# cvlab-stonybrook/s-volsdf

Measured on AMD Instinct MI355X. Metric: rendered rays/sec (1024-ray batch, 128 samples), higher is better.
Workload: dtype f32 (every product, forward and backward, as three fp16 MFMA products of two-piece fp16 operands with f32 accumulate; activation blocks hold both pieces: float32 accuracy class); 1 GPU; configs[1]: VolOpt.train_step (forward + MVS prior lookup + loss + backward + clip/guard/Adam), train mode, fast=1: 1024 rays/GPU x 128 coarse + 98 composited samples + 2048 eikonal points, 8x256 SDF MLP + 4x256 radiance MLP; mode=train, mlp_precision=fp16x2, launch=eager launches, rays_per_gpu=1024, rays_total=1024

## Files before the change

### s-volsdf_amd/csrc/svs_mlp_bwd_h2.hip

```cpp
#include "svs_mlp_h2_dev.h"
#include "svs_mlp_host.h"
#include "svs_mlp_bwd_args.h"
#include "svs_mlp_h2_trunk.h"
#include "svs_mlp_bwd_h2_dev.h"
#include "svs_ticket.h"
#include <cstdlib>

namespace svs {
namespace mlp {

template <bool GP>
struct RgbBwdEpi {
  f32x16 prev;
  TilePieces r;
  float v8[8];
  Pieces2* out;
  float* zblk;
  PointScale* ps;
  int lane;
  __device__ __forceinline__ void b(int tp, int rr) {
    float v = prev[rr] * ps->inv_in;
    v = hi_at(r, rr) > 0.0f ? v : 0.0f;
    pin(v);
    ps->track(v);
    v8[rr & 7] = v * ps->s_out;
    if ((rr & 7) == 7) {
      split8(v8, out->h[2 * tp + (rr >> 3)], out->m[2 * tp + (rr >> 3)]);
      pin(out->h[2 * tp + (rr >> 3)], out->m[2 * tp + (rr >> 3)]);
    }
    if (rr == 9) store_piece(zblk, 2 * tp, lane, out->h[2 * tp], 0);
    if (GP && rr == 11) store_piece(zblk, 2 * tp, lane, out->m[2 * tp], 1);
    if (rr == 15) store_grad<GP>(zblk, 2 * tp + 1, lane, out->h[2 * tp + 1], out->m[2 * tp + 1]);
  }
  __device__ __forceinline__ void all(int tp) {
#pragma unroll
    for (int rr = 0; rr < 16; ++rr) b(tp, rr);
  }
};

template <bool GP>
__device__ __forceinline__ void rgb_bwd_layer_h2(Stream& st, const Pieces2& in, Pieces2& out, const float* rblk, float* zblk,
                                                 float* zrec, PointScale& ps, int lane) {
  RgbBwdEpi<GP> ep;
  ep.out = &out; ep.zblk = zblk; ep.ps = &ps; ep.lane = lane;
  store_record(zrec, lane, ps.s_out, 0.0f);
  TilePieces rnext;
  load_tile_hi(rblk, 0, lane, rnext);
#pragma unroll
  for (int t = 0; t < 8; ++t) {
    const TilePieces rcur = rnext;
    auto rload = [&](int s) {
      if (t == 7) return;
      if (s == 10) rnext.h[0] = load_piece(rblk, 2 * (t + 1), lane);
      if (s == 12) rnext.h[1] = load_piece(rblk, 2 * (t + 1) + 1, lane);
    };
    f32x16 acc;
    if (t == 0) acc = tile_mma_h2_pf<16, kChunkF4>(st, in, lane, NoEpi(), NoEpi(), rload);
    else acc = tile_mma_h2_pf<16, kChunkF4>(st, in, lane, NoEpi(), [&](int s) { ep.b(t - 1, s); }, rload);
    ep.prev = acc; ep.r = rcur;
    constexpr int kSt = GP ? 4 : 2;
    if (t == 0) st.advance_keep<2>();
    else if (t < 7) st.advance_keep<2 + kSt>();
    else st.advance_keep<kSt>();
  }
  ep.all(7);
  ps.next();
}

template <bool GP>
__global__ __launch_bounds__(kThreads, 1) void rgb_bwd_h2_kernel(RgbBwdArgs a) {
  extern __shared__ __attribute__((aligned(16))) unsigned char smem[];
  Stream st;
  st.g = a.stream; st.buf = reinterpret_cast<f32x4*>(smem); st.cur = 1;
  const int lane = threadIdx.x & 63, half = lane >> 5, wave = threadIdx.x >> 6;
  const int wtile = blockIdx.x * kWaves + wave;
  const int p = wtile * kTilePts + (lane & 31);
  const bool livep = p < a.P;
  const int pc = livep ? p : a.P - 1;
  const size_t LS = block_stride();
  const float* rb = a.rbuf + (size_t)wtile * kBlockF;
  float* zb = a.zbuf + (size_t)wtile * kBlockF;
  const size_t T = (size_t)gridDim.x * kWaves;
  auto zrec = [&](int l) { return record_ptr(a.zbuf, 5, T, l, wtile); };

  st.prefetch<kW4TF4>();
  float dz[3];
  float m0 = 0.0f;
#pragma unroll
  for (int c = 0; c < 3; ++c) {
    const float o = a.rgb[3 * pc + c];
    dz[c] = (livep && half == 0) ? a.d_rgb[3 * pc + c] * o * (1.0f - o) : 0.0f;
    m0 = __builtin_fmaxf(m0, __builtin_fabsf(dz[c]));
  }
  m0 = __builtin_fmaxf(m0, __shfl_xor(m0, 32));
  PointScale ps;
  ps.start(m0, 0.0f);
  {
    float v8[8] = {dz[0] * ps.s_in, dz[1] * ps.s_in, dz[2] * ps.s_in, 0.0f, 0.0f, 0.0f, 0.0f, 0.0f};
    store_grad8<GP>(zb + 4 * LS, 0, lane, v8);
    store_record(zrec(4), lane, ps.s_in, m0);
  }
  st.advance();
  Pieces2 pa, pb;
  st.prefetch<kChunkF4>();
  {
    const f32x4* c = st.cur_buf();
    const float* r4 = rb + 3 * LS;
    float* z3 = zb + 3 * LS;
    store_record(zrec(3), lane, ps.s_out, 0.0f);
#pragma unroll
    for (int t = 0; t < 8; ++t) {
      TilePieces r;
      load_tile_hi(r4, t, lane, r);
      const f32x4 w = c[t * 64 + lane];
      f32x16 acc = (f32x16)(0.0f);
      acc = __builtin_amdgcn_mfma_f32_32x32x2f32(w[0], dz[0], acc, 0, 0, 0);
      acc = __builtin_amdgcn_mfma_f32_32x32x2f32(w[1], dz[1], acc, 0, 0, 0);
      acc = __builtin_amdgcn_mfma_f32_32x32x2f32(w[2], dz[2], acc, 0, 0, 0);
#pragma unroll
      for (int i = 0; i < 16; ++i) { acc[i] = hi_at(r, i) > 0.0f ? acc[i] : 0.0f; ps.track(acc[i]); }
      split_tile_scaled(acc, t, pa, ps.s_out);
      store_grad<GP>(z3, 2 * t, lane, pa.h[2 * t], pa.m[2 * t]);
      store_grad<GP>(z3, 2 * t + 1, lane, pa.h[2 * t + 1], pa.m[2 * t + 1]);
    }
  }
  ps.next();
  st.advance();
  rgb_bwd_layer_h2<GP>(st, pa, pb, rb + 2 * LS, zb + 2 * LS, zrec(2), ps, lane);
  rgb_bwd_layer_h2<GP>(st, pb, pa, rb + 1 * LS, zb + 1 * LS, zrec(1), ps, lane);
  rgb_bwd_layer_h2<GP>(st, pa, pb, rb, zb, zrec(0), ps, lane);
  float* fb = a.feat_bar + (size_t)wtile * kBlockF;
  float fmax = 0.0f;
  const float s_f = ps.s_out;
  {
    f32x16 prev;
    float v8[8];
    auto slice = [&](int tp, int r) {
      const float v = prev[r] * ps.inv_in;
      fmax = __builtin_fmaxf(fmax, __builtin_fabsf(v));
      v8[r & 7] = v * s_f;
      if ((r & 7) == 7) store_grad8<GP>(fb, 2 * tp + (r >> 3), lane, v8);
    };
#pragma unroll
    for (int t = 0; t < 9; ++t) {
      if (t < 8) st.prefetch<kChunkF4>();
      f32x16 acc;
      if (t == 0) acc = tile_mma_h2<16>(st.cur_buf(), pb, lane);
      else acc = tile_mma_h2<16>(st.cur_buf(), pb, lane, NoEpi(), [&](int s) { slice(t - 1, s); });
      if (t < 8) { prev = acc; st.advance(); }
      else if (half == 1 && livep) {
        a.d_normals[3 * p] = acc[4] * ps.inv_in; a.d_normals[3 * p + 1] = acc[5] * ps.inv_in;
        a.d_normals[3 * p + 2] = acc[6] * ps.inv_in;
      }
    }
  }
  fmax = __builtin_fmaxf(fmax, __shfl_xor(fmax, 32));
  store_record(record_ptr(a.feat_bar, 1, T, 0, wtile), lane, s_f, fmax);
  publish_max(a.absmax + 1, ps.gmax);
  publish_max(a.absmax + 2, fmax);
}

constexpr int kSpliceF = 20;

template <bool SPLIT, bool GP>
struct PassAEpi {
  f32x16 prev;
  TilePieces h;
  float v, s1;
  float v8[8];
  f16x8 up[2], uq[2];
  Pieces2* out;
  float* ublk;
  float* urec;
  PointScale* ps;
  const float* splice;
  float vm;
  int lane, half;
  bool l3;

  __device__ __forceinline__ void begin() {
    if (lane < 32) urec[lane] = ps->s_out;
    vm = 0.0f;
  }
  __device__ __forceinline__ void end() {
    vm = __builtin_fmaxf(vm, __shfl_xor(vm, 32));
    if (lane >= 32) urec[lane] = vm;
  }
  __device__ __forceinline__ void a(int r) {
    v = prev[r] * ps->inv_in;
    s1 = 1.0f - __builtin_amdgcn_exp2f(grad_times<GP>(h, r, -100.0f * 1.44269504088896341f));
    pin(v); pin(s1);
  }
  template <bool LATE = false>
  __device__ __forceinline__ void b(int tp, int r) {
    float u = v * s1;
    float w = __builtin_fabsf(v) * (100.0f - 100.0f * s1);
    if (tp == 6 && r >= 12 && l3) {
      const bool sp = half == 1 || r >= 13;
      const float us = splice[(16 + (r - 12)) * kThreads];
      u = sp ? us : u;
      w = sp ? 0.0f : w;
    }
    pin(u); pin(w);
    emit<LATE>(tp, r, u, w);
  }
  template <bool LATE = false>
  __device__ __forceinline__ void emit(int tp, int r, float u, float w) {
    vm = __builtin_fmaxf(vm, w);
    ps->track(u);
    v8[r & 7] = u * ps->s_out;
    if ((r & 7) == 7) {
      const int k = 2 * tp + (r >> 3), q = r >> 3;
      if (SPLIT) {
        split8(v8, out->h[k], out->m[k]);
        pin(out->h[k], out->m[k]);
        up[q] = out->h[k];
        if (GP) uq[q] = out->m[k];
      } else if (GP) {
        split8(v8, up[q], uq[q]);
      } else {
        up[q] = hi8(v8, 1.0f);
      }
      if (!LATE) store_grad<GP>(ublk, k, lane, up[q], uq[q]);
    }
  }
  __device__ __forceinline__ void store_slot(int tp, int s) {
    if (s == 9) store_piece(ublk, 2 * tp, lane, up[0], 0);
    if (GP && s == 11) store_piece(ublk, 2 * tp, lane, uq[0], 1);
    if (s == 15) store_grad<GP>(ublk, 2 * tp + 1, lane, up[1], uq[1]);
  }
  __device__ __forceinline__ void all(int tp) {
#pragma unroll
    for (int r = 0; r < 16; ++r) { a(r); b(tp, r); }
  }
  __device__ __forceinline__ void splice_tile7() {
#pragma unroll
    for (int r = 0; r < 16; ++r) emit(7, r, splice[r * kThreads], 0.0f);
  }
};

template <bool SPLIT, bool LAST, bool GP>
__device__ __forceinline__ void pass_a_layer_h2(Stream& st, const Pieces2& in, PassAEpi<SPLIT, GP>& ep, const float* hblk, int lane) {
  ep.begin();
#pragma unroll
  for (int t = 0; t < 8; ++t) {
    if (t == 7 && ep.l3) break;
    TilePieces hload;
    load_tile_grad<GP>(hblk, t, lane, hload);
    const bool fetch = !(LAST && t == 7);
    f32x16 acc;
    if (!fetch) acc = tile_mma_h2<16>(st.cur_buf(), in, lane, [&](int s) { ep.a(s); }, [&](int s) { ep.b(t - 1, s); });
    else if (t == 0) acc = tile_mma_h2_pf<16, kChunkF4>(st, in, lane, NoEpi(), NoEpi());
    else acc = tile_mma_h2_pf<16, kChunkF4>(st, in, lane, [&](int s) { ep.a(s); },
                                            [&](int s) { ep.template b<true>(t - 1, s); ep.store_slot(t - 1, s); });
    ep.prev = acc; ep.h = hload;
    if (fetch) {
      if (t == 0) st.advance();
      else st.advance_keep<GP ? 4 : 2>();
    }
  }
  if (ep.l3) { ep.all(6); ep.splice_tile7(); }
  else ep.all(7);
  ep.end();
  ep.ps->next();
}

template <bool GP>
__global__ __launch_bounds__(kThreads, 1) void sdf_bwd_a_h2_kernel(SdfBwdAArgs a) {
  extern __shared__ __attribute__((aligned(16))) unsigned char smem[];
  Stream st;
  st.g = a.stream; st.buf = reinterpret_cast<f32x4*>(smem); st.cur = 1;
  float* splice = reinterpret_cast<float*>(smem + kLdsBytes) + threadIdx.x;
  const int lane = threadIdx.x & 63, half = lane >> 5, wave = threadIdx.x >> 6;
  const int wtile = blockIdx.x * kWaves + wave;
  const int p = wtile * kTilePts + (lane & 31);
  const int pc = p < a.src.P ? p : a.src.P - 1;

  st.prefetch<kChunk0F4>();
  PointScale ps;
  Pieces2 pa, pb;
  const size_t LS = block_stride();
  const float* hb = a.hbuf + (size_t)wtile * kBlockF;
  float* ub = a.ubuf + (size_t)wtile * kBlockF;
  const size_t T = (size_t)gridDim.x * kWaves;
  auto urec = [&](int l) { return record_ptr(a.ubuf, 9, T, l, wtile); };
  {
    float x0, x1, x2;
    load_point(a.src, p, x0, x1, x2);
    PosEnc pe;
    pe.compute(x0, x1, x2);
    float nb[3] = {a.d_grad[3 * pc], a.d_grad[3 * pc + 1], a.d_grad[3 * pc + 2]};
    if (p >= a.src.P || (a.clamp_mask && a.clamp_mask[pc])) { nb[0] = nb[1] = nb[2] = 0.0f; }
    PosEnc u0;
    float m0 = 0.0f;
#pragma unroll
    for (int q = 0; q < 40; ++q) {
      float coef = 1.0f; int c = q;
      if (q >= 3 && q < kPeDim) {
        const int f = (q - 3) / 6, w = (q - 3) % 6;
        const float sc = (float)(1 << f);
        c = w < 3 ? w : w - 3;
        coef = w < 3 ? sc * pe.v[q + 3] : -sc * pe.v[q - 3];
      }
      u0.v[q] = q < kPeDim ? coef * nb[c < 3 ? c : 0] : 0.0f;
      m0 = __builtin_fmaxf(m0, __builtin_fabsf(u0.v[q]));
    }
    ps.start(m0, 0.0f);
#pragma unroll
    for (int r = 0; r < 16; ++r) splice[r * kThreads] = half ? u0.v[rho(r) + 4] : u0.v[rho(r)];
#pragma unroll
    for (int r = 12; r < 16; ++r) {
      const int k0 = rho(r) - 25, k1 = rho(r) + 4 - 25;
      const float s0 = k0 >= 0 ? u0.v[32 + (k0 >= 0 ? k0 : 0)] : 0.0f;
      splice[(16 + r - 12) * kThreads] = half ? u0.v[32 + k1] : s0;
    }
    PosEnc us;
#pragma unroll
    for (int q = 0; q < 40; ++q) us.v[q] = u0.v[q] * ps.s_in;
    split_pe(us, half, pa);
    float* pbk = a.pebuf + (size_t)wtile * kBlockF;
#pragma unroll
    for (int k = 0; k < 3; ++k) {
      f16x8 fh, fm;
      block_fragment<kPeDim>(u0.v, k, half, ps.s_in, fh, fm);
      store_grad<GP>(ub, k, lane, fh, fm);
      block_fragment<kPeDim>(pe.v, k, half, 1.0f, fh, fm);
      store_grad<GP>(pbk, k, lane, fh, fm);
    }
    store_record(urec(0), lane, ps.s_in, m0);
  }
  st.advance();

  {
    PassAEpi<true, GP> ep;
    ep.out = &pb; ep.ublk = ub + LS; ep.urec = urec(1); ep.ps = &ps; ep.splice = splice;
    ep.lane = lane; ep.half = half; ep.l3 = false;
    ep.begin();
#pragma unroll
    for (int t = 0; t < 8; ++t) {
      TilePieces hload;
      load_tile_grad<GP>(hb, t, lane, hload);
      if (t < 7) st.prefetch<kChunk0F4>(); else st.prefetch<kChunkF4>();
      const f32x16 acc = tile_mma_h2<3>(st.cur_buf(), pa, lane);
      if (t > 0) ep.all(t - 1);
      ep.prev = acc; ep.h = hload;
      st.advance();
    }
    ep.all(7);
    ep.end();
    ps.next();
  }
  for (int l = 1; l < 7; ++l) {
    PassAEpi<true, GP> ep;
    ep.out = &pa; ep.ublk = ub + (size_t)(l + 1) * LS; ep.urec = urec(l + 1);
    ep.ps = &ps; ep.splice = splice; ep.lane = lane; ep.half = half; ep.l3 = l == 3;
    pass_a_layer_h2<true, false, GP>(st, pb, ep, hb + (size_t)l * LS, lane);
#pragma unroll
    for (int s = 0; s < 16; ++s) { pb.h[s] = pa.h[s]; pb.m[s] = pa.m[s]; }
  }
  {
    PassAEpi<false, GP> ep;
    ep.out = nullptr; ep.ublk = ub + (size_t)8 * LS; ep.urec = urec(8);
    ep.ps = &ps; ep.splice = splice; ep.lane = lane; ep.half = half; ep.l3 = false;
    pass_a_layer_h2<false, true, GP>(st, pb, ep, hb + (size_t)7 * LS, lane);
  }
  publish_max(a.absmax, ps.gmax);
}

template <bool FIRST, bool SPLIT, typename Net, bool A2, bool GP>
struct PassBEpi {
  static constexpr bool kG = A2 || FIRST;
  f32x16 prev;
  TilePieces h, u, g;
  float v, s1, q;
  float v8[8];
  f16x8 ap[2], aq[2];
  Pieces2* out;
  float* ablk;
  float* arec;
  PointScale* ps;
  float sbar, u_inv100;
  int lane, half;
  bool l4;
  __device__ __forceinline__ void a(int r) {
    v = prev[r] * ps->inv_in;
    float e = __builtin_amdgcn_exp2f(grad_times<GP>(h, r, -100.0f * 1.44269504088896341f));
    if (A2) e = __builtin_fminf(e, 0.99999994f);
    s1 = 1.0f - e;
    if (A2) q = e * u_inv100;
    pin(v); pin(s1);
    if (A2) pin(q);
  }
  template <bool LATE = false>
  __device__ __forceinline__ void b(int tp, int r) {
    float o = v * s1;
    if (A2) {
      const float gg = grad_mix<GP>(g, r);
      const float t = grad_times<GP>(u, r, gg);
      o = __builtin_fmaf(t, q * __builtin_amdgcn_rcpf(s1), o);
      if (FIRST) o = __builtin_fmaf(sbar, gg, o);
    } else if (FIRST) {
      o = __builtin_fmaf(sbar, grad_mix<GP>(g, r), o);
    }
    if (l4 && tp > Net::kSpliceTile) o = 0.0f;
    if (l4 && tp == Net::kSpliceTile) {
      const bool z0 = rho(r) >= Net::kSpliceLocal, z1 = rho(r) + 4 >= Net::kSpliceLocal;
      if (z0 || z1) { if (half ? z1 : z0) o = 0.0f; }
    }
    pin(o);
    ps->track(o);
    v8[r & 7] = o * ps->s_out;
    if ((r & 7) == 7) {
      const int k = 2 * tp + (r >> 3), q2 = r >> 3;
      if (SPLIT) {
        split8(v8, out->h[k], out->m[k]);
        pin(out->h[k], out->m[k]);
        ap[q2] = out->h[k];
        if (GP) aq[q2] = out->m[k];
      } else if (GP) {
        split8(v8, ap[q2], aq[q2]);
      } else {
        ap[q2] = hi8(v8, 1.0f);
      }
      if (!LATE) store_grad<GP>(ablk, k, lane, ap[q2], aq[q2]);
    }
  }
  __device__ __forceinline__ void store_slot(int tp, int s) {
    if (s == 9) store_grad<GP>(ablk, 2 * tp, lane, ap[0], aq[0]);
    if (s == 15) store_grad<GP>(ablk, 2 * tp + 1, lane, ap[1], aq[1]);
  }
  __device__ __forceinline__ void all(int tp) {
#pragma unroll
    for (int r = 0; r < 16; ++r) { a(r); b(tp, r); }
  }
};

template <bool FIRST, bool SPLIT, bool LAST_STAGE, typename Net, bool A2, bool GP>
__device__ __forceinline__ void pass_b_stage_h2(Stream& st, const Pieces2& in, PassBEpi<FIRST, SPLIT, Net, A2, GP>& ep, const float* hblk,
                                                const float* ublk, const float* urec, const float* gblk, float next_floor, int lane) {
  constexpr bool kG = A2 || FIRST;
  store_record(ep.arec, lane, ep.ps->s_out, 0.0f);
  ep.u_inv100 = A2 ? 100.0f * PointScale::inv_pow2(load_scale(urec, lane)) : 0.0f;
  TilePieces hnext, unext, gnext;
  load_tile_grad<GP>(hblk, 0, lane, hnext);
  if (A2) load_tile_grad<GP>(ublk, 0, lane, unext);
  if (kG) load_tile_grad<GP>(gblk, 0, lane, gnext);
  constexpr int kPer = GP ? 4 : 2;
  constexpr int kLoads = kPer * (1 + (A2 ? 1 : 0) + (kG ? 1 : 0));
  constexpr int kStores = GP ? 4 : 2;
#pragma unroll
  for (int t = 0; t < 8; ++t) {
    const TilePieces hcur = hnext, ucur = unext, gcur = gnext;
    auto side = [&](int s) {
      if (t == 7) return;
      if (s == 10) hnext.h[0] = load_piece(hblk, 2 * (t + 1), lane);
      if (s == 11) hnext.h[1] = load_piece(hblk, 2 * (t + 1) + 1, lane);
      if (A2 && s == 12) unext.h[0] = load_piece(ublk, 2 * (t + 1), lane);
      if (A2 && s == 13) unext.h[1] = load_piece(ublk, 2 * (t + 1) + 1, lane);
      if (kG && s == 14) gnext.h[0] = load_piece(gblk, 2 * (t + 1), lane);
      if (kG && s == 15) gnext.h[1] = load_piece(gblk, 2 * (t + 1) + 1, lane);
      if (GP) {
        if (s == 10) hnext.m[0] = load_piece(hblk, 2 * (t + 1), lane, 1);
        if (s == 11) hnext.m[1] = load_piece(hblk, 2 * (t + 1) + 1, lane, 1);
        if (A2 && s == 12) unext.m[0] = load_piece(ublk, 2 * (t + 1), lane, 1);
        if (A2 && s == 13) unext.m[1] = load_piece(ublk, 2 * (t + 1) + 1, lane, 1);
        if (kG && s == 14) gnext.m[0] = load_piece(gblk, 2 * (t + 1), lane, 1);
        if (kG && s == 15) gnext.m[1] = load_piece(gblk, 2 * (t + 1) + 1, lane, 1);
      }
    };
    const bool fetch = !(LAST_STAGE && t == 7);
    f32x16 acc;
    if (!fetch) acc = tile_mma_h2<16>(st.cur_buf(), in, lane, [&](int s) { ep.a(s); }, [&](int s) { ep.b(t - 1, s); });
    else if (t == 0) acc = tile_mma_h2_pf<16, kChunkF4>(st, in, lane, NoEpi(), NoEpi(), side);
    else acc = tile_mma_h2_pf<16, kChunkF4>(st, in, lane, [&](int s) { ep.a(s); },
                                            [&](int s) { ep.template b<true>(t - 1, s); ep.store_slot(t - 1, s); }, side);
    ep.prev = acc; ep.h = hcur;
    if (A2) ep.u = ucur;
    if (kG) ep.g = gcur;
    if (fetch) {
      if (t == 0) st.advance_keep<kLoads>();
      else if (t < 7) st.advance_keep<kLoads + kStores>();
      else st.advance_keep<kStores>();
    }
  }
  ep.all(7);
  ep.ps->floor_m = next_floor;
  ep.ps->next();
}

template <typename Net, bool A2, bool GP>
__global__ __launch_bounds__(kThreads, 1) void sdf_bwd_b_h2_kernel(SdfBwdBArgs a) {
  extern __shared__ __attribute__((aligned(16))) unsigned char smem[];
  Stream st;
  st.g = a.stream; st.buf = reinterpret_cast<f32x4*>(smem); st.cur = 1;
  const int lane = threadIdx.x & 63, half = lane >> 5, wave = threadIdx.x >> 6;
  const int bx = a.reverse ? (int)(gridDim.x - 1 - blockIdx.x) : (int)blockIdx.x;
  const int wtile = bx * kWaves + wave;
  const int p = wtile * kTilePts + (lane & 31);
  const int pc = p < a.P ? p : a.P - 1;
  st.prefetch<kChunkF4>();
  float sbar = (a.d_sdf && p < a.P) ? a.d_sdf[pc] : 0.0f;
  if (a.clamp_mask && a.clamp_mask[pc]) sbar = 0.0f;
  if (half == 0 && a.sbar_out) a.sbar_out[p] = sbar;
  const size_t LS = block_stride();
  const float* hb = a.hbuf + (size_t)wtile * kBlockF;
  const float* gb = A2 ? a.gbuf + (size_t)wtile * kBlockF : a.w0 + (size_t)wtile * a.w0_stride - 7 * LS;
  const float* ub = A2 ? a.ubuf + (size_t)wtile * kBlockF : nullptr;
  float* ab = a.abuf + (size_t)wtile * kBlockF;
  const size_t T = (size_t)gridDim.x * kWaves;
  auto arec = [&](int l) { return record_ptr(a.abuf, 8, T, l, wtile); };
  auto urec = [&](int l) { return A2 ? record_ptr(a.ubuf, 9, T, l, wtile) : nullptr; };
  const float asb = __builtin_fabsf(sbar);
  auto floor_of = [&](int l) {
    return A2 ? __builtin_fmaxf(asb, load_max(urec(l + 1), lane) * load_max(record_ptr(a.gbuf, 8, T, l, wtile), lane)) : asb;
  };
  const bool has_f = a.feat_bar && wtile < a.n_feat_tiles;
  PointScale ps;
  Pieces2 pa, pb;
  {
    const float fl = floor_of(7);
    if (has_f) {
      const float* fb = a.feat_bar + (size_t)wtile * kBlockF;
      const float* frec = record_ptr(a.feat_bar, 1, (size_t)((a.n_feat_tiles + kWaves - 1) / kWaves * kWaves), 0, wtile);
#pragma unroll
      for (int k = 0; k < 16; ++k) {
        pa.h[k] = load_piece(fb, k, lane);
        pa.m[k] = GP ? load_piece(fb, k, lane, 1) : (f16x8)(_Float16)0.0f;
      }
      ps.start_stored(load_scale(frec, lane), load_max(frec, lane), fl);
    } else {
#pragma unroll
      for (int k = 0; k < 16; ++k) { pa.h[k] = (f16x8)(_Float16)0.0f; pa.m[k] = (f16x8)(_Float16)0.0f; }
      ps.start(0.0f, fl);
    }
    ps.gmax = 0.0f;
  }
  st.advance();
  {
    PassBEpi<true, true, Net, A2, GP> ep;
    ep.out = &pb; ep.ablk = ab + 7 * LS; ep.arec = arec(7); ep.ps = &ps; ep.sbar = sbar; ep.lane = lane; ep.half = half; ep.l4 = false;
    pass_b_stage_h2<true, true, false, Net, A2, GP>(st, pa, ep, hb + 7 * LS, A2 ? ub + 8 * LS : nullptr, urec(8), gb + 7 * LS,
                                                    floor_of(6), lane);
  }
  for (int l = 7; l >= 2; --l) {
    PassBEpi<false, true, Net, A2, GP> ep;
    ep.out = &pa; ep.ablk = ab + (size_t)(l - 1) * LS; ep.arec = arec(l - 1); ep.ps = &ps; ep.sbar = 0.0f; ep.lane = lane; ep.half = half;
    ep.l4 = l == 4;
    pass_b_stage_h2<false, true, false, Net, A2, GP>(st, pb, ep, hb + (size_t)(l - 1) * LS, A2 ? ub + (size_t)l * LS : nullptr, urec(l),
                                                     A2 ? gb + (size_t)(l - 1) * LS : nullptr, floor_of(l >= 2 ? l - 2 : 0), lane);
#pragma unroll
    for (int s = 0; s < 16; ++s) { pb.h[s] = pa.h[s]; pb.m[s] = pa.m[s]; }
  }
  {
    PassBEpi<false, false, Net, A2, GP> ep;
    ep.out = nullptr; ep.ablk = ab; ep.arec = arec(0); ep.ps = &ps; ep.sbar = 0.0f; ep.lane = lane; ep.half = half; ep.l4 = false;
    pass_b_stage_h2<false, false, true, Net, A2, GP>(st, pb, ep, hb, A2 ? ub + LS : nullptr, urec(1), A2 ? gb : nullptr, asb, lane);
  }
  publish_max(a.absmax, ps.gmax);
}

template <bool GP>
__global__ __launch_bounds__(256) void lin8_row0_h2_kernel(const float* __restrict__ hbuf, const float* __restrict__ ubuf,
                                                           const float* __restrict__ sbar, int n_tiles, int n_tiles_pad, int P,
                                                           float* __restrict__ out, det::Ticket ticket) {
  __shared__ float red[4][32][65];
  const int lane = threadIdx.x & 63, quarter = threadIdx.x >> 6;
  float acc[32];
#pragma unroll
  for (int i = 0; i < 32; ++i) acc[i] = 0.0f;
  float bsum = 0.0f;
  for (int t = blockIdx.x; t < n_tiles; t += gridDim.x) {
    const int p = t * 32 + (lane & 31);
    const float sb = p < P ? sbar[p] : 0.0f;
    const float* h = hbuf + ((size_t)7 * n_tiles_pad + t) * kBlockF;
    f16x8 hh[4], hm[4], uh[4], um[4];
    float us = 0.0f;
#pragma unroll
    for (int k = 0; k < 4; ++k) { hh[k] = load_piece(h, 4 * quarter + k, lane, 0); hm[k] = load_piece(h, 4 * quarter + k, lane, 1); }
    if (ubuf) {
      const float* u = ubuf + ((size_t)8 * n_tiles_pad + t) * kBlockF;
#pragma unroll
      for (int k = 0; k < 4; ++k) {
        uh[k] = load_piece(u, 4 * quarter + k, lane);
        um[k] = GP ? load_piece(u, 4 * quarter + k, lane, 1) : (f16x8)(_Float16)0.0f;
      }
      us = p < P ? PointScale::inv_pow2(load_scale(record_ptr(ubuf, 9, (size_t)n_tiles_pad, 8, t), lane)) : 0.0f;
    } else {
#pragma unroll
      for (int k = 0; k < 4; ++k) { uh[k] = (f16x8)(_Float16)0.0f; um[k] = (f16x8)(_Float16)0.0f; }
    }
#pragma unroll
    for (int k = 0; k < 4; ++k)
#pragma unroll
      for (int j = 0; j < 8; ++j)
        acc[8 * k + j] += sb * ((float)hh[k][j] + (float)hm[k][j]) + us * ((float)uh[k][j] + (float)um[k][j]);
    if (quarter == 0 && lane < 32) bsum += sb;
  }
#pragma unroll
  for (int i = 0; i < 32; ++i) red[quarter][i][lane] = acc[i];
  __syncthreads();
  det::wait_turn(ticket, blockIdx.x);
  {
    const int q = threadIdx.x >> 6, i = (threadIdx.x >> 1) & 31, hf = threadIdx.x & 1;
    float v = 0.0f;
#pragma unroll 8
    for (int c = 0; c < 32; ++c) v += red[q][i][32 * hf + c];
    const int k = i >> 3, j = i & 7;
    atomicAdd(&out[16 * (4 * q + k) + 8 * (j >> 2) + 4 * hf + (j & 3)], v);
  }
  if (quarter == 0) {
    for (int d = 16; d >= 1; d >>= 1) bsum += __shfl_xor(bsum, d);
    if (lane == 0) atomicAdd(&out[256], bsum);
  }
  det::pass_turn(ticket, blockIdx.x);
}

int launch_lin8_row0_h2(const float* hbuf, const float* ubuf, const float* sbar, int n_points, int n_tiles_pad, float* out257,
                        bool gp, hipStream_t s) {
  const int n_tiles = (n_points + 31) / 32;
  const int grid = n_tiles < 256 ? n_tiles : 256;
  const det::Ticket ticket{det::take_slots(1), 0u, (unsigned)grid};
  if (gp) lin8_row0_h2_kernel<true><<<grid, 256, 0, s>>>(hbuf, ubuf, sbar, n_tiles, n_tiles_pad, n_points, out257, ticket);
  else lin8_row0_h2_kernel<false><<<grid, 256, 0, s>>>(hbuf, ubuf, sbar, n_tiles, n_tiles_pad, n_points, out257, ticket);
  return check_launch("svs_lin8_row0_grad");
}

int launch_rgb_bwd_h2(const RgbBwdArgs& a, bool gp, hipStream_t s) {
  static int once = set_lds(rgb_bwd_h2_kernel<true>, kLdsBytes, "svs_rgb_bwd") | set_lds(rgb_bwd_h2_kernel<false>, kLdsBytes, "svs_rgb_bwd");
  if (once) return once;
  const int grid = (a.P + kWgPts - 1) / kWgPts;
  if (gp) rgb_bwd_h2_kernel<true><<<grid, kThreads, kLdsBytes, s>>>(a);
  else rgb_bwd_h2_kernel<false><<<grid, kThreads, kLdsBytes, s>>>(a);
  return check_launch("svs_rgb_bwd");
}
int launch_sdf_bwd_a_h2(const SdfBwdAArgs& a, bool gp, hipStream_t s) {
  constexpr int lds = kLdsBytes + kSpliceF * kThreads * (int)sizeof(float);
  static int once = set_lds(sdf_bwd_a_h2_kernel<true>, lds, "svs_sdf_bwd_a") | set_lds(sdf_bwd_a_h2_kernel<false>, lds, "svs_sdf_bwd_a");
  if (once) return once;
  const int grid = (a.src.P + kWgPts - 1) / kWgPts;
  if (gp) sdf_bwd_a_h2_kernel<true><<<grid, kThreads, lds, s>>>(a);
  else sdf_bwd_a_h2_kernel<false><<<grid, kThreads, lds, s>>>(a);
  return check_launch("svs_sdf_bwd_a");
}
int launch_sdf_bwd_b_h2(const SdfBwdBArgs& a_in, bool gp, hipStream_t s) {
  static int once = set_lds(sdf_bwd_b_h2_kernel<NetFg, true, true>, kLdsBytes, "svs_sdf_bwd_b") |
                    set_lds(sdf_bwd_b_h2_kernel<NetFg, true, false>, kLdsBytes, "svs_sdf_bwd_b");
  if (once) return once;
  static const int reverse_env = [] { const char* e = getenv("SVS_BWD_B_REVERSE"); return e ? atoi(e) : 0; }();
  SdfBwdBArgs a = a_in;
  a.reverse = reverse_env;
  const int grid = (a.P + kWgPts - 1) / kWgPts;
  if (gp) sdf_bwd_b_h2_kernel<NetFg, true, true><<<grid, kThreads, kLdsBytes, s>>>(a);
  else sdf_bwd_b_h2_kernel<NetFg, true, false><<<grid, kThreads, kLdsBytes, s>>>(a);
  return check_launch("svs_sdf_bwd_b");
}
int launch_bg_bwd_b_h2(const SdfBwdBArgs& a, bool gp, hipStream_t s) {
  static int once = set_lds(sdf_bwd_b_h2_kernel<NetBg, false, true>, kLdsBytes, "svs_bg_sdf_bwd") |
                    set_lds(sdf_bwd_b_h2_kernel<NetBg, false, false>, kLdsBytes, "svs_bg_sdf_bwd");
  if (once) return once;
  const int grid = (a.P + kWgPts - 1) / kWgPts;
  if (gp) sdf_bwd_b_h2_kernel<NetBg, false, true><<<grid, kThreads, kLdsBytes, s>>>(a);
  else sdf_bwd_b_h2_kernel<NetBg, false, false><<<grid, kThreads, kLdsBytes, s>>>(a);
  return check_launch("svs_bg_sdf_bwd");
}

}
}
```

### s-volsdf_amd/csrc/svs_mlp_bwd_h2_dev.h

```cpp
#pragma once
#include "svs_mlp_h2_dev.h"
#include "svs_blocks_h2.h"

namespace svs {
namespace mlp {

struct PointScale {
  float s_in, inv_in;
  float s_out;
  float m;
  float floor_m;
  float gmax;

  static __device__ __forceinline__ float pow2_for(float mx) {
    int e = (int)((__float_as_uint(mx) >> 23) & 0xff);
    e = e < 24 ? 24 : (e > 230 ? 230 : e);
    return __uint_as_float((unsigned)(258 - e) << 23);
  }
  static __device__ __forceinline__ float inv_pow2(float s) { return __uint_as_float((254u << 23) - __float_as_uint(s)); }
  __device__ __forceinline__ void start(float m0, float fl) {
    floor_m = fl; gmax = m0;
    s_in = pow2_for(__builtin_fmaxf(m0, fl)); inv_in = inv_pow2(s_in);
    s_out = s_in; m = 0.0f;
  }
  __device__ __forceinline__ void start_stored(float s_stored, float m0, float fl) {
    floor_m = fl; gmax = m0;
    s_in = s_stored; inv_in = inv_pow2(s_in);
    s_out = pow2_for(__builtin_fmaxf(m0, fl)); m = 0.0f;
  }
  __device__ __forceinline__ void track(float v) { m = __builtin_fmaxf(m, __builtin_fabsf(v)); }
  __device__ __forceinline__ void next() {
    m = __builtin_fmaxf(m, __shfl_xor(m, 32));
    gmax = __builtin_fmaxf(gmax, m);
    s_in = s_out; inv_in = inv_pow2(s_in);
    s_out = pow2_for(__builtin_fmaxf(m, floor_m));
    m = 0.0f;
  }
};

__device__ __forceinline__ void publish_max(float* slot, float v) {
#pragma unroll
  for (int d = 32; d >= 1; d >>= 1) v = __builtin_fmaxf(v, __shfl_xor(v, d));
  if ((threadIdx.x & 63) == 0) atomicMax(reinterpret_cast<unsigned*>(slot), __float_as_uint(v));
}

__device__ __forceinline__ void split_tile_scaled(const f32x16& y, int t, Pieces2& p, float s) {
  f32x16 v;
#pragma unroll
  for (int r = 0; r < 16; ++r) v[r] = y[r] * s;
  split_tile(v, t, p);
}

}
}
```

### s-volsdf_amd/csrc/svs_mlp_h2_dev.h

```cpp
#pragma once
#include "svs_mlp_dev.h"

namespace svs {
namespace mlp {

typedef _Float16 f16x8 __attribute__((ext_vector_type(8)));

struct Pieces2 {
  f16x8 h[18], m[18];
};

__device__ __forceinline__ void split8(const float* v, f16x8& h, f16x8& m) {
#pragma unroll
  for (int j = 0; j < 8; ++j) {
    const _Float16 ah = (_Float16)v[j];
    h[j] = ah;
    m[j] = (_Float16)(v[j] - (float)ah);
  }
}

__device__ __forceinline__ void pin(float& v) { asm volatile("" : "+v"(v)); }
__device__ __forceinline__ void pin(f16x8& a, f16x8& b) { asm volatile("" : "+v"(a), "+v"(b)); }

__device__ __forceinline__ void split_tile(const f32x16& y, int t, Pieces2& p) {
#pragma unroll
  for (int s = 0; s < 2; ++s) {
    float v[8];
#pragma unroll
    for (int j = 0; j < 8; ++j) v[j] = y[8 * s + j];
    split8(v, p.h[2 * t + s], p.m[2 * t + s]);
  }
}

template <int KS, int PAD>
__device__ __forceinline__ void split_pe(const float* pev, int half, Pieces2& p) {
#pragma unroll
  for (int s = 0; s < KS; ++s) {
    float v[8];
#pragma unroll
    for (int j = 0; j < 8; ++j) {
      const int q0 = 16 * s + j, q1 = 16 * s + 8 + j;
      const float a0 = q0 < PAD ? pev[q0 < PAD ? q0 : 0] : 0.0f;
      const float a1 = q1 < PAD ? pev[q1 < PAD ? q1 : 0] : 0.0f;
      v[j] = half ? a1 : a0;
    }
    split8(v, p.h[s], p.m[s]);
  }
}
__device__ __forceinline__ void split_pe(const PosEnc& pe, int half, Pieces2& p) { split_pe<3, 40>(pe.v, half, p); }

__device__ __forceinline__ f32x16 tile_bias(const f32x4* __restrict__ chunk, int lane) {
  f32x16 acc;
#pragma unroll
  for (int r4 = 0; r4 < 4; ++r4) {
    const f32x4 b = chunk[r4 * 64 + lane];
    acc[4 * r4 + 0] = b[0]; acc[4 * r4 + 1] = b[1]; acc[4 * r4 + 2] = b[2]; acc[4 * r4 + 3] = b[3];
  }
  return acc;
}

struct NoEpi { __device__ __forceinline__ void operator()(int) const {} };
struct NoPre { __device__ __forceinline__ void operator()() const {} };

template <int KS, typename EpiA, typename EpiB, typename Dma = NoEpi, typename EpiC = NoEpi, typename Pre = NoPre>
__device__ __forceinline__ f32x16 tile_mma_h2(const f32x4* __restrict__ chunk, const Pieces2& x, int lane, EpiA ea, EpiB eb,
                                              int first_step = 0, Dma dma = Dma(), EpiC ec = EpiC(), Pre pre = Pre()) {
  f32x16 acc = tile_bias(chunk, lane);
  const f16x8* a_ptr = reinterpret_cast<const f16x8*>(chunk + kHdrF4) + lane;
  f16x8 ah = a_ptr[0], am = a_ptr[64];
  __builtin_amdgcn_sched_barrier(0);
  pre();
#pragma unroll
  for (int s = 0; s < KS; ++s) {
    f16x8 nh, nm;
    __builtin_amdgcn_sched_barrier(0);
    acc = __builtin_amdgcn_mfma_f32_32x32x16_f16(am, x.h[first_step + s], acc, 0, 0, 0);
    __builtin_amdgcn_sched_barrier(0);
    if (s + 1 < KS) { nh = a_ptr[(2 * s + 2) * 64]; nm = a_ptr[(2 * s + 3) * 64]; }
    ea(s);
    __builtin_amdgcn_sched_barrier(0);
    acc = __builtin_amdgcn_mfma_f32_32x32x16_f16(ah, x.m[first_step + s], acc, 0, 0, 0);
    __builtin_amdgcn_sched_barrier(0);
    eb(s);
    __builtin_amdgcn_sched_barrier(0);
    acc = __builtin_amdgcn_mfma_f32_32x32x16_f16(ah, x.h[first_step + s], acc, 0, 0, 0);
    __builtin_amdgcn_sched_barrier(0);
    ec(s);
    dma(s);
    if (s + 1 < KS) { ah = nh; am = nm; }
  }
  return acc;
}
template <int KS>
__device__ __forceinline__ f32x16 tile_mma_h2(const f32x4* __restrict__ chunk, const Pieces2& x, int lane) {
  return tile_mma_h2<KS>(chunk, x, lane, NoEpi(), NoEpi());
}

template <int KS, int N16, typename S, typename EpiA, typename EpiB, typename EpiC = NoEpi, typename Pre = NoPre>
__device__ __forceinline__ f32x16 tile_mma_h2_pf(S& st, const Pieces2& x, int lane, EpiA ea, EpiB eb, EpiC ec = EpiC(),
                                                 Pre pre = Pre()) {
  const f32x16 acc = tile_mma_h2<KS>(st.cur_buf(), x, lane, ea, eb, 0, [&](int s) { st.template prefetch_step<N16, KS>(s); }, ec,
                                     pre);
  st.template prefetch_done<N16>();
  return acc;
}

struct SoftplusA { float mx, lg; };
__device__ __forceinline__ float softplus100_b(const SoftplusA& r) {
  return r.mx + (0.69314718055994531f / 100.0f) * r.lg;
}

}
}
```

Baseline: 299,500 rays/s.

## Pipeline feat_bar layer weight prefetch and hoist rgb layer-4 activation loads

The final feat_bar GEMM layer in the RGB backward kernel now uses the prefetching MMA path, overlapping the next weight chunk load with the current tile's MFMAs, and its epilogue stores are spread across late MFMA steps through a new FeatBarEpi. The first layer's ReLU-mask activation tiles and the rgb/d_rgb inputs are all loaded up front, before the scale setup, instead of inside the per-tile loop. Store scheduling is factored into shared helpers (store_tile_late, kTileStores), and the stream advance counts now account for outstanding stores. This is meant to hide global-memory latency, at the cost of more live registers (8 hoisted tiles) and more complex wait-count bookkeeping.

Result: faster. 302,700 rays/s (median of 6 runs) (+1.1%).

```diff
diff --git a/s-volsdf_amd/csrc/svs_mlp_bwd_h2.hip b/s-volsdf_amd/csrc/svs_mlp_bwd_h2.hip
--- a/s-volsdf_amd/csrc/svs_mlp_bwd_h2.hip
+++ b/s-volsdf_amd/csrc/svs_mlp_bwd_h2.hip
@@ -28,9 +28,7 @@
       split8(v8, out->h[2 * tp + (rr >> 3)], out->m[2 * tp + (rr >> 3)]);
       pin(out->h[2 * tp + (rr >> 3)], out->m[2 * tp + (rr >> 3)]);
     }
-    if (rr == 9) store_piece(zblk, 2 * tp, lane, out->h[2 * tp], 0);
-    if (GP && rr == 11) store_piece(zblk, 2 * tp, lane, out->m[2 * tp], 1);
-    if (rr == 15) store_grad<GP>(zblk, 2 * tp + 1, lane, out->h[2 * tp + 1], out->m[2 * tp + 1]);
+    store_tile_late<GP>(zblk, tp, lane, rr, &out->h[2 * tp], &out->m[2 * tp]);
   }
   __device__ __forceinline__ void all(int tp) {
 #pragma unroll
@@ -58,7 +56,7 @@
     if (t == 0) acc = tile_mma_h2_pf<16, kChunkF4>(st, in, lane, NoEpi(), NoEpi(), rload);
     else acc = tile_mma_h2_pf<16, kChunkF4>(st, in, lane, NoEpi(), [&](int s) { ep.b(t - 1, s); }, rload);
     ep.prev = acc; ep.r = rcur;
-    constexpr int kSt = GP ? 4 : 2;
+    constexpr int kSt = kTileStores<GP>;
     if (t == 0) st.advance_keep<2>();
     else if (t < 7) st.advance_keep<2 + kSt>();
     else st.advance_keep<kSt>();
@@ -66,6 +64,28 @@
   ep.all(7);
   ps.next();
 }
+
+template <bool GP>
+struct FeatBarEpi {
+  f32x16 prev;
+  float v8[8];
+  f16x8 fh[2], fm[2];
+  float* fblk;
+  float inv_in, s_f;
+  float fmax;
+  int lane;
+  __device__ __forceinline__ void b(int tp, int r) {
+    float v = prev[r] * inv_in;
+    pin(v);
+    fmax = __builtin_fmaxf(fmax, __builtin_fabsf(v));
+    v8[r & 7] = v * s_f;
+    if ((r & 7) == 7) {
+      if (GP) { split8(v8, fh[r >> 3], fm[r >> 3]); pin(fh[r >> 3], fm[r >> 3]); }
+      else { fh[r >> 3] = hi8(v8, 1.0f); pin(fh[r >> 3]); }
+    }
+    store_tile_late<GP>(fblk, tp, lane, r, fh, fm);
+  }
+};
 
 template <bool GP>
 __global__ __launch_bounds__(kThreads, 1) void rgb_bwd_h2_kernel(RgbBwdArgs a) {
@@ -84,12 +104,19 @@
   auto zrec = [&](int l) { return record_ptr(a.zbuf, 5, T, l, wtile); };
 
   st.prefetch<kW4TF4>();
+  TilePieces r4t[8];
+#pragma unroll
+  for (int t = 0; t < 8; ++t) load_tile_hi(rb + 3 * LS, t, lane, r4t[t]);
+  float o3[3], g3[3];
+#pragma unroll
+  for (int c = 0; c < 3; ++c) { o3[c] = a.rgb[3 * pc + c]; g3[c] = a.d_rgb[3 * pc + c]; }
+  __builtin_amdgcn_sched_barrier(0);
   float dz[3];
   float m0 = 0.0f;
 #pragma unroll
   for (int c = 0; c < 3; ++c) {
-    const float o = a.rgb[3 * pc + c];
-    dz[c] = (livep && half == 0) ? a.d_rgb[3 * pc + c] * o * (1.0f - o) : 0.0f;
+    const float o = o3[c];
+    dz[c] = (livep && half == 0) ? g3[c] * o * (1.0f - o) : 0.0f;
     m0 = __builtin_fmaxf(m0, __builtin_fabsf(dz[c]));
   }
   m0 = __builtin_fmaxf(m0, __shfl_xor(m0, 32));
@@ -101,17 +128,17 @@
     store_record(zrec(4), lane, ps.s_in, m0);
   }
   st.advance();
+#pragma unroll
+  for (int t = 0; t < 8; ++t) pin(r4t[t].h[0], r4t[t].h[1]);
   Pieces2 pa, pb;
   st.prefetch<kChunkF4>();
   {
     const f32x4* c = st.cur_buf();
-    const float* r4 = rb + 3 * LS;
     float* z3 = zb + 3 * LS;
     store_record(zrec(3), lane, ps.s_out, 0.0f);
 #pragma unroll
     for (int t = 0; t < 8; ++t) {
-      TilePieces r;
-      load_tile_hi(r4, t, lane, r);
+      const TilePieces& r = r4t[t];
       const f32x4 w = c[t * 64 + lane];
       f32x16 acc = (f32x16)(0.0f);
       acc = __builtin_amdgcn_mfma_f32_32x32x2f32(w[0], dz[0], acc, 0, 0, 0);
@@ -120,42 +147,35 @@
 #pragma unroll
       for (int i = 0; i < 16; ++i) { acc[i] = hi_at(r, i) > 0.0f ? acc[i] : 0.0f; ps.track(acc[i]); }
       split_tile_scaled(acc, t, pa, ps.s_out);
-      store_grad<GP>(z3, 2 * t, lane, pa.h[2 * t], pa.m[2 * t]);
-      store_grad<GP>(z3, 2 * t + 1, lane, pa.h[2 * t + 1], pa.m[2 * t + 1]);
+      store_tile_pieces<GP>(z3, t, lane, &pa.h[2 * t], &pa.m[2 * t]);
     }
   }
   ps.next();
-  st.advance();
+  st.advance_keep<8 * kTileStores<GP>>();
   rgb_bwd_layer_h2<GP>(st, pa, pb, rb + 2 * LS, zb + 2 * LS, zrec(2), ps, lane);
   rgb_bwd_layer_h2<GP>(st, pb, pa, rb + 1 * LS, zb + 1 * LS, zrec(1), ps, lane);
   rgb_bwd_layer_h2<GP>(st, pa, pb, rb, zb, zrec(0), ps, lane);
-  float* fb = a.feat_bar + (size_t)wtile * kBlockF;
-  float fmax = 0.0f;
-  const float s_f = ps.s_out;
-  {
-    f32x16 prev;
-    float v8[8];
-    auto slice = [&](int tp, int r) {
-      const float v = prev[r] * ps.inv_in;
-      fmax = __builtin_fmaxf(fmax, __builtin_fabsf(v));
-      v8[r & 7] = v * s_f;
-      if ((r & 7) == 7) store_grad8<GP>(fb, 2 * tp + (r >> 3), lane, v8);
-    };
+  FeatBarEpi<GP> ep;
+  ep.fblk = a.feat_bar + (size_t)wtile * kBlockF; ep.inv_in = ps.inv_in; ep.s_f = ps.s_out; ep.fmax = 0.0f; ep.lane = lane;
+  {
 #pragma unroll
     for (int t = 0; t < 9; ++t) {
-      if (t < 8) st.prefetch<kChunkF4>();
       f32x16 acc;
-      if (t == 0) acc = tile_mma_h2<16>(st.cur_buf(), pb, lane);
-      else acc = tile_mma_h2<16>(st.cur_buf(), pb, lane, NoEpi(), [&](int s) { slice(t - 1, s); });
-      if (t < 8) { prev = acc; st.advance(); }
-      else if (half == 1 && livep) {
+      if (t == 0) acc = tile_mma_h2_pf<16, kChunkF4>(st, pb, lane, NoEpi(), NoEpi());
+      else if (t < 8) acc = tile_mma_h2_pf<16, kChunkF4>(st, pb, lane, NoEpi(), [&](int s) { ep.b(t - 1, s); });
+      else acc = tile_mma_h2<16>(st.cur_buf(), pb, lane, NoEpi(), [&](int s) { ep.b(t - 1, s); });
+      if (t < 8) {
+        ep.prev = acc;
+        if (t == 0) st.advance();
+        else st.advance_keep<kTileStores<GP>>();
+      } else if (half == 1 && livep) {
         a.d_normals[3 * p] = acc[4] * ps.inv_in; a.d_normals[3 * p + 1] = acc[5] * ps.inv_in;
         a.d_normals[3 * p + 2] = acc[6] * ps.inv_in;
       }
     }
   }
-  fmax = __builtin_fmaxf(fmax, __shfl_xor(fmax, 32));
-  store_record(record_ptr(a.feat_bar, 1, T, 0, wtile), lane, s_f, fmax);
+  const float fmax = __builtin_fmaxf(ep.fmax, __shfl_xor(ep.fmax, 32));
+  store_record(record_ptr(a.feat_bar, 1, T, 0, wtile), lane, ep.s_f, fmax);
   publish_max(a.absmax + 1, ps.gmax);
   publish_max(a.absmax + 2, fmax);
 }
@@ -256,7 +276,7 @@
     ep.prev = acc; ep.h = hload;
     if (fetch) {
       if (t == 0) st.advance();
-      else st.advance_keep<GP ? 4 : 2>();
+      else st.advance_keep<kTileStores<GP>>();
     }
   }
   if (ep.l3) { ep.all(6); ep.splice_tile7(); }
@@ -447,7 +467,7 @@
   if (kG) load_tile_grad<GP>(gblk, 0, lane, gnext);
   constexpr int kPer = GP ? 4 : 2;
   constexpr int kLoads = kPer * (1 + (A2 ? 1 : 0) + (kG ? 1 : 0));
-  constexpr int kStores = GP ? 4 : 2;
+  constexpr int kStores = kTileStores<GP>;
 #pragma unroll
   for (int t = 0; t < 8; ++t) {
     const TilePieces hcur = hnext, ucur = unext, gcur = gnext;
diff --git a/s-volsdf_amd/csrc/svs_mlp_bwd_h2_dev.h b/s-volsdf_amd/csrc/svs_mlp_bwd_h2_dev.h
--- a/s-volsdf_amd/csrc/svs_mlp_bwd_h2_dev.h
+++ b/s-volsdf_amd/csrc/svs_mlp_bwd_h2_dev.h
@@ -44,6 +44,30 @@
   if ((threadIdx.x & 63) == 0) atomicMax(reinterpret_cast<unsigned*>(slot), __float_as_uint(v));
 }
 
+template <bool GP>
+constexpr int kTileStores = GP ? 4 : 2;
+template <bool GP>
+__device__ __forceinline__ void store_tile_piece(float* blk, int tp, int lane, int i, const f16x8* h, const f16x8* m) {
+  const int f = GP ? i >> 1 : i;
+  if (GP && (i & 1)) store_piece(blk, 2 * tp + f, lane, m[f], 1);
+  else store_piece(blk, 2 * tp + f, lane, h[f], 0);
+}
+template <bool GP>
+__device__ __forceinline__ void store_tile_pieces(float* blk, int tp, int lane, const f16x8* h, const f16x8* m) {
+#pragma unroll
+  for (int i = 0; i < kTileStores<GP>; ++i) store_tile_piece<GP>(blk, tp, lane, i, h, m);
+}
+template <bool GP>
+__device__ __forceinline__ constexpr int late_store_step(int i) {
+  return (GP ? i >> 1 : i) ? 15 : ((GP && (i & 1)) ? 11 : 9);
+}
+template <bool GP>
+__device__ __forceinline__ void store_tile_late(float* blk, int tp, int lane, int s, const f16x8* h, const f16x8* m) {
+#pragma unroll
+  for (int i = 0; i < kTileStores<GP>; ++i)
+    if (s == late_store_step<GP>(i)) store_tile_piece<GP>(blk, tp, lane, i, h, m);
+}
+
 __device__ __forceinline__ void split_tile_scaled(const f32x16& y, int t, Pieces2& p, float s) {
   f32x16 v;
 #pragma unroll
diff --git a/s-volsdf_amd/csrc/svs_mlp_h2_dev.h b/s-volsdf_amd/csrc/svs_mlp_h2_dev.h
--- a/s-volsdf_amd/csrc/svs_mlp_h2_dev.h
+++ b/s-volsdf_amd/csrc/svs_mlp_h2_dev.h
@@ -20,6 +20,7 @@
 }
 
 __device__ __forceinline__ void pin(float& v) { asm volatile("" : "+v"(v)); }
+__device__ __forceinline__ void pin(f16x8& a) { asm volatile("" : "+v"(a)); }
 __device__ __forceinline__ void pin(f16x8& a, f16x8& b) { asm volatile("" : "+v"(a), "+v"(b)); }
 
 __device__ __forceinline__ void split_tile(const f32x16& y, int t, Pieces2& p) {
```
